# jondeaton/PhaMers

Hardware: AMD Instinct MI355X
Metric: Gbases/s k-mer-count+score, k=4, 5 kb contigs (higher is better)
Workload: dtype u32 counts + f16 MFMA proposal (exact integer counts x fp16 reference parts, f32 accumulate; k=4: high parts in the sweep, low parts added in f64 to the window's candidates) + f64 decision; 1 GPU; BASELINE configs[1]: k=4, 1000000 x 5000-base contigs per GPU, count+normalise+combo score, 4510 reference rows + 172 centroids; contigs_per_gpu=1000000, contig_length=5000, k=4, method=combo, parallelism=contig shards, 1 rank(s), replicated reference, final all-gather of scores

## Files before the change

### phamers_amd/csrc/count_slots.hip

```cpp
#include "count_shared.h"


__global__ __launch_bounds__(256) void phk_count_plan_kernel(const uint64_t *__restrict__ offsets, uint64_t n, int k,
                                                             uint32_t gs,
                                                             uint32_t long_thr, uint32_t piece_w, int sort,
                                                             uint32_t *__restrict__ ctl, uint32_t *__restrict__ ctl_next,
                                                             uint32_t *__restrict__ z0, uint32_t z0n, uint32_t *__restrict__ z1, uint32_t z1n) {
    __shared__ uint32_t h[SORT_KEYS];
    __shared__ unsigned long long s_pad[4], s_used[4];
    __shared__ uint32_t s_last;
    const int tid = threadIdx.x;
    {
        const uint32_t g0 = blockIdx.x * 256u + (uint32_t)tid, gn = gridDim.x * 256u;
        for (uint32_t i = g0; i < (uint32_t)CTL_WORDS; i += gn) ctl_next[i] = 0;
        for (uint32_t i = g0; i < z0n; i += gn) z0[i] = 0;
        for (uint32_t i = g0; i < z1n; i += gn) z1[i] = 0;
    }
    if (sort)
        for (int i = tid; i < SORT_KEYS; i += 256) h[i] = 0;
    __syncthreads();
    unsigned long long pad = 0, used = 0;
    for (uint64_t base = (uint64_t)blockIdx.x * PLAN_PER_BLOCK; base < n; base += (uint64_t)gridDim.x * PLAN_PER_BLOCK) {
        uint64_t o0[PLAN_PER_BLOCK / 256], o1[PLAN_PER_BLOCK / 256];
#pragma unroll
        for (int it = 0; it < PLAN_PER_BLOCK / 256; ++it) {
            const uint64_t c = base + (uint64_t)it * 256 + tid;
            const uint64_t cc = c < n ? c : n - 1;
            o0[it] = offsets[cc];
            o1[it] = offsets[cc + 1];
        }
#pragma unroll
        for (int it = 0; it < PLAN_PER_BLOCK / 256; ++it) {
            const uint64_t c = base + (uint64_t)it * 256 + tid;
            const bool have = c < n;
            uint64_t w = 0;
            if (have) {
                const uint64_t len = o1[it] - o0[it];
                w = len >= (uint64_t)k ? len - k + 1 : 0;
            }
            const unsigned long long wq = (have && w <= long_thr) ? w : 0ull;
            used += wq;
            unsigned long long mx = wq;
            for (uint32_t sft = 1; sft < gs; sft <<= 1) {
                const unsigned long long o = __shfl_xor(mx, (int)sft);
                mx = o > mx ? o : mx;
            }
            if (have && (c % gs) == 0) pad += (unsigned long long)gs * (((mx + 1023) >> 10) << 10);
            if (sort) {
                const uint32_t np = (have && w > long_thr && piece_w) ? (uint32_t)((w + piece_w - 1) / piece_w) : 1u;
                const uint32_t key = phk_windows_key(phk_piece_windows(w, np, np - 1, piece_w));
                const unsigned long long live = __ballot(have);
                const uint32_t key0 = __builtin_amdgcn_readfirstlane(key);
                if (__all(!have || (key == key0 && np == 1)) && (live & 1ull)) {
                    if ((tid & 63) == 0) atomicAdd(&h[key0], (uint32_t)__popcll(live));
                } else if (have) {
                    if (np > 1) atomicAdd(&h[phk_windows_key(piece_w)], np - 1);
                    atomicAdd(&h[key], 1u);
                }
            }
        }
    }
#pragma unroll
    for (int sft = 32; sft > 0; sft >>= 1) {
        pad += __shfl_xor(pad, sft);
        used += __shfl_xor(used, sft);
    }
    if ((tid & 63) == 0) {
        s_pad[tid >> 6] = pad;
        s_used[tid >> 6] = used;
    }
    __syncthreads();
    unsigned long long *stats = reinterpret_cast<unsigned long long *>(ctl + CTL_STATS);
    if (tid == 0) {
        pad = s_pad[0] + s_pad[1] + s_pad[2] + s_pad[3];
        used = s_used[0] + s_used[1] + s_used[2] + s_used[3];
        if (pad) {
            atomicAdd(stats, pad);
            atomicAdd(stats + 1, used);
        }
    }
    if (sort)
        for (int i = tid; i < SORT_KEYS; i += 256)
            if (h[i]) atomicAdd(ctl + CTL_CURSOR + i, h[i]);
    asm volatile("s_waitcnt vmcnt(0)" ::: "memory");
    __syncthreads();
    if (tid == 0) s_last = atomicAdd(ctl + CTL_TICKET, 1u) == gridDim.x - 1 ? 1u : 0u;
    __syncthreads();
    if (!s_last || !sort) return;
    const unsigned long long pad_t = __hip_atomic_load(stats, __ATOMIC_RELAXED, __HIP_MEMORY_SCOPE_AGENT);
    const unsigned long long used_t = __hip_atomic_load(stats + 1, __ATOMIC_RELAXED, __HIP_MEMORY_SCOPE_AGENT);
    if (used_t * 10ull >= pad_t * 6ull) return;
    for (int i = tid; i < SORT_KEYS; i += 256)
        h[i] = __hip_atomic_load(ctl + CTL_CURSOR + (SORT_KEYS - 1 - i), __ATOMIC_RELAXED, __HIP_MEMORY_SCOPE_AGENT);
    __syncthreads();
    if (tid < 64) {
        uint32_t loc = 0;
        for (int i = 0; i < SORT_KEYS / 64; ++i) loc += h[tid * (SORT_KEYS / 64) + i];
        uint32_t inc = loc;
#pragma unroll
        for (int sft = 1; sft < 64; sft <<= 1) {
            const uint32_t o = __shfl_up(inc, sft);
            if (tid >= sft) inc += o;
        }
        uint32_t run = inc - loc;
        for (int i = 0; i < SORT_KEYS / 64; ++i) {
            const uint32_t cnt = h[tid * (SORT_KEYS / 64) + i];
            h[tid * (SORT_KEYS / 64) + i] = run;
            run += cnt;
        }
        if (tid == 63) ctl[CTL_ITEMS] = run;
    }
    __syncthreads();
    for (int i = tid; i < SORT_KEYS; i += 256) ctl[CTL_CURSOR + (SORT_KEYS - 1 - i)] = h[i];
}

__global__ __launch_bounds__(256) void phk_sort_scatter_kernel(const uint64_t *__restrict__ offsets, uint64_t n, int k,
                                                               uint32_t long_thr, uint32_t piece_w,
                                                               const unsigned long long *__restrict__ stats,
                                                               uint32_t *__restrict__ cursor, uint2 *__restrict__ items,
                                                               uint32_t *__restrict__ counts, uint32_t *__restrict__ nwin) {
    if (phk_slots_apply(stats)) return;
    __shared__ uint32_t h[SORT_KEYS];
    const uint64_t per_block = (n + gridDim.x - 1) / gridDim.x;
    const uint64_t lo = per_block * blockIdx.x, hi = lo + per_block < n ? lo + per_block : n;
    const uint64_t D = 1ull << (2 * k);
    for (int i = threadIdx.x; i < SORT_KEYS; i += blockDim.x) h[i] = 0;
    __syncthreads();
    for (uint64_t c = lo + threadIdx.x; c < hi; c += blockDim.x) {
        uint32_t np;
        const uint64_t w = phk_contig_windows(offsets, c, k, long_thr, piece_w, np);
        if (np > 1) atomicAdd(&h[phk_windows_key(piece_w)], np - 1);
        atomicAdd(&h[phk_windows_key(phk_piece_windows(w, np, np - 1, piece_w))], 1u);
    }
    __syncthreads();
    for (int i = threadIdx.x; i < SORT_KEYS; i += blockDim.x)
        if (h[i]) h[i] = atomicAdd(cursor + i, h[i]);
    __syncthreads();
    for (uint64_t c = lo + threadIdx.x; c < hi; c += blockDim.x) {
        uint32_t np;
        const uint64_t w = phk_contig_windows(offsets, c, k, long_thr, piece_w, np);
        for (uint32_t pc = 0; pc < np; ++pc)
            items[atomicAdd(&h[phk_windows_key(phk_piece_windows(w, np, pc, piece_w))], 1u)] = make_uint2((uint32_t)c, pc);
        if (np > 1) {
            uint4 *row = reinterpret_cast<uint4 *>(counts + c * D);
            for (uint64_t i = 0; i < D / 4; ++i) row[i] = make_uint4(0, 0, 0, 0);
            if (nwin) nwin[c] = 0;
        }
    }
}


template <int NTH>
__global__ __launch_bounds__(NTH) void phk_count_pairs_kernel(const uint32_t *__restrict__ packed, const uint64_t *__restrict__ offsets,
                                                             uint64_t n, uint64_t max_word, uint32_t long_thr,
                                                             uint32_t *__restrict__ counts, uint32_t *__restrict__ nwin,
                                                             uint2 *__restrict__ long_list, uint32_t *__restrict__ long_count,
                                                             uint32_t piece_w) {
    constexpr int K = 4;
    constexpr uint32_t D = 256, NWORD = 512;
    constexpr int SLOTS = 32;
    constexpr int PARTS = NTH / SLOTS;
    constexpr int XPT = (int)D / PARTS;
    static_assert(XPT % 4 == 0, "flush geometry");
    extern __shared__ __attribute__((aligned(16))) uint32_t lds[];
    uint32_t *single_s = lds + NWORD * SLOTS;
    if (!phk_slots_apply(reinterpret_cast<const unsigned long long *>(long_count + CTL_STATS))) return;
    const int t = threadIdx.x;
    const int slot = t & (SLOTS - 1), part = t / SLOTS;
    for (uint32_t b = t * 4; b < NWORD * SLOTS; b += 4 * NTH) *reinterpret_cast<uint4 *>(lds + b) = make_uint4(0, 0, 0, 0);
    __syncthreads();
    const uint32_t colb = (uint32_t)slot * 4u;
    const uint32_t pthr = long_thr < 131070u ? long_thr : 131070u;
    typedef __attribute__((address_space(3))) uint32_t lds_u32;
    auto pair_addr = [&](uint32_t src, int o) { return (lds_u32 *)(uintptr_t)(((src >> (16 - 2 * o)) & (0x1FFu << 7)) | colb); };
    auto pair_inc = [&](uint32_t src, int o) {
        uint32_t bit, inc;
        asm("v_bfe_u32 %0, %1, %2, 1" : "=v"(bit) : "v"(src), "n"(22 - 2 * o));
        asm("v_mad_u32_u24 %0, %1, %2, 1" : "=v"(inc) : "v"(bit), "v"(65535u));
        return inc;
    };
#if defined(PHK_DIAGNOSTIC_BUILD) && defined(PAIRS_ABL) && PAIRS_ABL == 1
    auto add1 = [&](lds_u32 *p, uint32_t val) { asm volatile("" ::"v"(p), "v"(val)); };
#else
    auto add1 = [&](lds_u32 *p, uint32_t val) { __hip_atomic_fetch_add(p, val, __ATOMIC_RELAXED, __HIP_MEMORY_SCOPE_WORKGROUP); };
#endif
    const uint64_t wlast = max_word + 1;

    for (uint64_t batch = blockIdx.x; batch * SLOTS < n; batch += gridDim.x) {
        const uint64_t c = batch * SLOTS + slot;
        const bool have = c < n;
        const uint64_t st = have ? offsets[c] : 0;
        const uint64_t en = have ? offsets[c + 1] : 0;
        const uint64_t len = en - st;
        uint32_t W = len >= (uint64_t)K ? (uint32_t)((len - K + 1) < 0xFFFFFFFFull ? (len - K + 1) : 0xFFFFFFFFull) : 0;
        const bool handed_over = W > pthr;
        if (handed_over) {
            if (part == 0) {
                const uint32_t np = piece_w ? (W + piece_w - 1) / piece_w : 1u;
                const uint32_t base = atomicAdd(long_count, np);
                for (uint32_t pc = 0; pc < np; ++pc) long_list[base + pc] = make_uint2((uint32_t)c, pc);
            }
            W = 0;
        }
        const uint32_t par = (uint32_t)st & 1u;
        const uint32_t npair = W >> 1;
        const uint64_t U0 = st >> 6;
        const uint32_t rst = (uint32_t)(st - (U0 << 6));
        const uint32_t rPL = rst + 2u * npair - 2u;
        const uint32_t nunit = npair ? (rPL >> 6) + 1u : 0u;
        const uint32_t *pc = packed + 4 * U0;
        const uint32_t wlim = (uint32_t)((wlast - 4 * U0) < 0x7FFFFFFFull ? (wlast - 4 * U0) : 0x7FFFFFFFull);
        if (part == 0) {
            uint32_t sg = 0xFFFFFFFFu;
            if (W & 1u) {
                const uint64_t lb = st + W - 1, wl = lb >> 4;
                const uint64_t f = ((uint64_t)packed[wl] << 32) | packed[wl + 1];
                sg = (uint32_t)(f >> (56 - 2 * (uint32_t)(lb & 15))) & 0xFFu;
            }
            single_s[slot] = sg;
        }
        auto load5 = [&](uint32_t j, uint32_t (&w)[5]) {
            const uint32_t w0 = 4u * j;
            if (w0 + 3 <= wlim) {
                const uint4 a = *reinterpret_cast<const uint4 *>(pc + w0);
                w[0] = a.x; w[1] = a.y; w[2] = a.z; w[3] = a.w;
            } else {
                w[0] = pc[w0]; w[1] = pc[w0 + 1 < wlim ? w0 + 1 : wlim]; w[2] = pc[w0 + 2 < wlim ? w0 + 2 : wlim]; w[3] = pc[wlim];
            }
            w[4] = pc[w0 + 4 < wlim ? w0 + 4 : wlim];
        };
        uint32_t cur[5] = {0, 0, 0, 0, 0}, nxt[5] = {0, 0, 0, 0, 0};
        uint32_t j = (uint32_t)part;
        if (j < nunit) load5(j, cur);
        while (__any(j < nunit)) {
            const bool live = j < nunit;
            if (j + PARTS < nunit) load5(j + PARTS, nxt);
            const uint32_t s0 = 64u * j + par;
            const bool all = live && s0 >= rst && s0 + 62u <= rPL;
            uint32_t sw[5];
#pragma unroll
            for (int i = 0; i < 4; ++i) sw[i] = par ? __builtin_amdgcn_alignbit(cur[i], cur[i + 1], 30) : cur[i];
            sw[4] = par ? cur[4] << 2 : cur[4];
            if (!__any(live && !all)) {
                if (all) {
#pragma unroll
                    for (int wd = 0; wd < 4; ++wd) {
                        const uint32_t y = sw[wd], u = __builtin_amdgcn_alignbit(y, sw[wd + 1], 16);
#pragma unroll
                        for (int jp = 0; jp < 8; ++jp) {
                            const uint32_t src = jp < 5 ? y : u;
                            const int o = jp < 5 ? 2 * jp : 2 * jp - 8;
                            add1(pair_addr(src, o), pair_inc(src, o));
                        }
                    }
                }
            } else if (live) {
                const uint32_t ilo = rst > s0 ? (rst - s0) >> 1 : 0u;
                const uint32_t ihi = (rPL - s0) >> 1 < 31u ? (rPL - s0) >> 1 : 31u;
                const uint32_t pm = (ihi - ilo == 31u) ? ~0u : (((1u << (ihi - ilo + 1)) - 1u) << (31 - ihi));
#pragma unroll
                for (int wd = 0; wd < 4; ++wd) {
                    const uint32_t y = sw[wd], u = __builtin_amdgcn_alignbit(y, sw[wd + 1], 16);
#pragma unroll
                    for (int jp = 0; jp < 8; ++jp) {
                        const uint32_t src = jp < 5 ? y : u;
                        const int o = jp < 5 ? 2 * jp : 2 * jp - 8;
                        add1(pair_addr(src, o), pair_inc(src, o) * __builtin_amdgcn_ubfe(pm, 31 - (8 * wd + jp), 1));
                    }
                }
            }
#pragma unroll
            for (int i = 0; i < 5; ++i) cur[i] = nxt[i];
            j += PARTS;
        }
        phk_lds_barrier();
        {
            const uint32_t x0 = (uint32_t)part * XPT;
            uint32_t out[XPT];
            const uint32_t *col = lds + slot;
#pragma unroll
            for (int i = 0; i < XPT; ++i) {
                const uint32_t w0 = col[(2 * (x0 + i)) * SLOTS], w1 = col[(2 * (x0 + i) + 1) * SLOTS];
                out[i] = __builtin_amdgcn_sad_u16(w1, 0u, __builtin_amdgcn_sad_u16(w0, 0u, 0u));
            }
            const uint32_t one = 1u;
#pragma unroll
            for (int mm = 0; mm < XPT / 2; ++mm)
#pragma unroll
                for (int a = 0; a < 4; ++a) {
                    const uint32_t w = col[(128 * a + x0 / 2 + mm) * SLOTS];
                    asm("v_mad_u32_u16 %0, %1, %2, %0" : "+v"(out[2 * mm]) : "v"(w), "v"(one));
                    asm("v_mad_u32_u16 %0, %1, %2, %0 op_sel:[1,0,0,0]" : "+v"(out[2 * mm + 1]) : "v"(w), "v"(one));
                }
            const uint32_t sg = single_s[slot];
#pragma unroll
            for (int i = 0; i < XPT; ++i) out[i] += (sg == x0 + i) ? 1u : 0u;
            phk_lds_barrier();
            uint32_t *zc = lds + (2 * x0) * SLOTS + slot;
#pragma unroll
            for (int i = 0; i < 2 * XPT; ++i) zc[i * SLOTS] = 0;
            uint32_t *rowo = counts + c * D + x0;
#if defined(PHK_DIAGNOSTIC_BUILD) && defined(PAIRS_ABL) && PAIRS_ABL == 2
            if (have && (!handed_over || piece_w) && (batch & 63) == 0) {
#else
            if (have && (!handed_over || piece_w)) {
#endif
#pragma unroll
                for (int i = 0; i < XPT / 4; ++i)
                    *reinterpret_cast<uint4 *>(rowo + 4 * i) = make_uint4(out[4 * i], out[4 * i + 1], out[4 * i + 2], out[4 * i + 3]);
            }
            if (nwin && have && part == 0 && (!handed_over || piece_w)) nwin[c] = W;
        }
        phk_lds_barrier();
    }
}

template <int K, int SLOTS, int NTH, bool MASK, bool ORDERED>
__global__ __launch_bounds__(NTH) void phk_count_direct_kernel(const uint32_t *__restrict__ packed, const uint32_t *__restrict__ mask,
                                                              const uint64_t *__restrict__ offsets,
                                                              uint64_t n, uint64_t max_word, uint32_t long_thr,
                                                              uint32_t *__restrict__ counts, uint32_t *__restrict__ nwin,
                                                              uint2 *__restrict__ long_list, uint32_t *__restrict__ long_count,
                                                              const uint2 *__restrict__ order,
                                                              uint32_t piece_w,
                                                              uint32_t skip_plain,
                                                              uint4 *__restrict__ frag8,
                                                              uint32_t *__restrict__ big8) {
    constexpr uint32_t D = 1u << (2 * K);
    constexpr int PARTS = NTH / SLOTS;
    constexpr int XPT = (int)D / PARTS;
    constexpr int SHB = SLOTS == 32 ? 7 : 6;
    static_assert(XPT % 4 == 0 && K <= 5, "flush geometry / window fits the funnel");
    extern __shared__ __attribute__((aligned(16))) uint32_t lds[];
    uint32_t *nwin_s = lds + D * SLOTS;
    uint32_t *split_s = nwin_s + SLOTS;
    const bool plain = phk_slots_apply(reinterpret_cast<const unsigned long long *>(long_count + CTL_STATS));
    if (ORDERED) {
        if (plain || !order) return;
        n = long_count[CTL_ITEMS];
        frag8 = nullptr;
        big8 = nullptr;
    } else {
        if (!plain) {
            if (big8 && blockIdx.x == 0 && threadIdx.x == 0) big8[n] = 2u;
            return;
        }
        if (skip_plain) return;
        order = nullptr;
    }
    const int t = threadIdx.x;
    const int slot = t & (SLOTS - 1), part = t / SLOTS;
    for (uint32_t b = t * 4; b < D * SLOTS; b += 4 * NTH) *reinterpret_cast<uint4 *>(lds + b) = make_uint4(0, 0, 0, 0);
    if (t < SLOTS) nwin_s[t] = 0;
    __syncthreads();
    const uint32_t colb = (uint32_t)slot * 4u;
    typedef __attribute__((address_space(3))) uint32_t lds_u32;
    auto bin = [&](uint32_t src, int o) {
        constexpr uint32_t msk = (D - 1u) << SHB;
        const int sh = 32 - 2 * K - 2 * o - SHB;
        return (lds_u32 *)(uintptr_t)(((src >> sh) & msk) | colb);
    };
    auto add1 = [&](lds_u32 *p, uint32_t val) { __hip_atomic_fetch_add(p, val, __ATOMIC_RELAXED, __HIP_MEMORY_SCOPE_WORKGROUP); };
    const uint64_t wlast = max_word + 1;
    const uint64_t mlast = (max_word >> 1) + 1;

    for (uint64_t batch = blockIdx.x; batch * SLOTS < n; batch += gridDim.x) {
        const uint64_t ci = batch * SLOTS + slot;
        const bool have = ci < n;
        const uint2 item = (ORDERED && have) ? order[ci] : make_uint2(0, 0);
        const uint64_t c = have ? (ORDERED ? (uint64_t)item.x : ci) : 0;
        uint64_t st = have ? offsets[c] : 0;
        const uint64_t en = have ? offsets[c + 1] : 0;
        const uint64_t len = en - st;
        uint32_t W = len >= (uint64_t)K ? (uint32_t)((len - K + 1) < 0xFFFFFFFFull ? (len - K + 1) : 0xFFFFFFFFull) : 0;
        const bool split = ORDERED && piece_w && W > long_thr;
        if (split) {
            const uint64_t first = (uint64_t)item.y * piece_w;
            st += first;
            W = (uint32_t)((uint64_t)W - first < piece_w ? (uint64_t)W - first : piece_w);
        }
        const bool handed_over = !ORDERED && W > long_thr;
        if (ORDERED && part == 0) split_s[slot] = split ? (uint32_t)c + 1u : 0u;
        if (handed_over) {
            if (part == 0) {
                const uint32_t np = piece_w ? (W + piece_w - 1) / piece_w : 1u;
                const uint32_t base = atomicAdd(long_count, np);
                for (uint32_t pc = 0; pc < np; ++pc) long_list[base + pc] = make_uint2((uint32_t)c, pc);
            }
            W = 0;
        }
        const uint64_t U0 = st >> 6;
        const uint32_t rst = (uint32_t)(st - (U0 << 6));
        const uint64_t rlast64 = (uint64_t)rst + W - 1;
        const uint32_t rlast = rlast64 < 0xFFFFFFC0ull ? (uint32_t)rlast64 : 0xFFFFFFC0u;
        const uint32_t nunit = W ? (rlast >> 6) + 1u : 0u;
        const uint32_t *pc = packed + 4 * U0;
        const uint32_t wlim = (uint32_t)((wlast - 4 * U0) < 0x7FFFFFFFull ? (wlast - 4 * U0) : 0x7FFFFFFFull);
        const uint32_t *pm = MASK ? mask + 2 * U0 : nullptr;
        const uint32_t mlim = MASK ? (uint32_t)((mlast - 2 * U0) < 0x7FFFFFFFull ? (mlast - 2 * U0) : 0x7FFFFFFFull) : 0u;
        auto load5 = [&](uint32_t j, uint32_t (&w)[5], uint32_t (&mk)[3]) {
            const uint32_t w0 = 4u * j;
            if (w0 + 3 <= wlim) {
                const uint4 a = *reinterpret_cast<const uint4 *>(pc + w0);
                w[0] = a.x; w[1] = a.y; w[2] = a.z; w[3] = a.w;
            } else {
                w[0] = pc[w0]; w[1] = pc[w0 + 1 < wlim ? w0 + 1 : wlim]; w[2] = pc[w0 + 2 < wlim ? w0 + 2 : wlim]; w[3] = pc[wlim];
            }
            w[4] = pc[w0 + 4 < wlim ? w0 + 4 : wlim];
            if (MASK) {
#pragma unroll
                for (int i = 0; i < 3; ++i) mk[i] = pm[2 * j + i < mlim ? 2 * j + i : mlim];
            }
        };
        uint32_t cur[5] = {0, 0, 0, 0, 0}, nxt[5] = {0, 0, 0, 0, 0}, mcur[3] = {0, 0, 0}, mnxt[3] = {0, 0, 0};
        uint32_t cnt_ok = 0;
        uint32_t j = (uint32_t)part;
        if (j < nunit) load5(j, cur, mcur);
        while (__any(j < nunit)) {
            const bool live = j < nunit;
            if (j + PARTS < nunit) load5(j + PARTS, nxt, mnxt);
            const uint32_t fb = 64u * j;
            bool all = live && fb >= rst && fb + 63u <= rlast;
            uint64_t wv = 0;
            if (MASK ? live : (live && !all)) {
                const uint32_t lo = rst > fb ? rst - fb : 0u;
                const uint32_t hi = rlast - fb < 63u ? rlast - fb : 63u;
                wv = (hi - lo == 63u) ? ~0ull : (((1ull << (hi - lo + 1)) - 1ull) << (63 - hi));
                if (MASK) {
                    const uint64_t vb = ((uint64_t)mcur[0] << 32) | mcur[1];
                    uint64_t w = vb;
#pragma unroll
                    for (int jj = 1; jj < K; ++jj) w &= (vb << jj) | ((uint64_t)mcur[2] >> (32 - jj));
                    wv &= w;
                    all = all && w == ~0ull;
                    cnt_ok += (uint32_t)__popcll(wv);
                }
            }
            if (!__any(live && !all)) {
                if (all) {
#pragma unroll
                    for (int wd = 0; wd < 4; ++wd) {
                        const uint32_t y = cur[wd], u = __builtin_amdgcn_alignbit(y, cur[wd + 1], 16);
#pragma unroll
                        for (int jw = 0; jw < 16; ++jw) add1(bin(jw < 8 ? y : u, jw & 7), 1u);
                    }
                }
            } else if (live) {
                if (!MASK && all) wv = ~0ull;
                const uint32_t vhi = (uint32_t)(wv >> 32), vlo = (uint32_t)wv;
#pragma unroll
                for (int wd = 0; wd < 4; ++wd) {
                    const uint32_t y = cur[wd], u = __builtin_amdgcn_alignbit(y, cur[wd + 1], 16);
#pragma unroll
                    for (int jw = 0; jw < 16; ++jw) {
                        const int wi = 16 * wd + jw;
                        add1(bin(jw < 8 ? y : u, jw & 7), __builtin_amdgcn_ubfe(wi < 32 ? vhi : vlo, 31 - (wi & 31), 1));
                    }
                }
            }
#pragma unroll
            for (int i = 0; i < 5; ++i) cur[i] = nxt[i];
            if (MASK) {
#pragma unroll
                for (int i = 0; i < 3; ++i) mcur[i] = mnxt[i];
            }
            j += PARTS;
        }
        if (MASK && cnt_ok) atomicAdd(nwin_s + slot, cnt_ok);
        phk_lds_barrier();
        if (ORDERED) {
            for (int sl = t >> 6; sl < SLOTS; sl += NTH / 64) {
                const uint32_t cs = split_s[sl];
                if (!cs) continue;
                uint32_t *rowp = counts + (uint64_t)(cs - 1u) * D;
                for (uint32_t code = (uint32_t)(t & 63); code < D; code += 64) {
                    const uint32_t v = lds[code * SLOTS + sl];
                    if (v) atomicAdd(rowp + code, v);
                }
            }
            phk_lds_barrier();
        }
        {
            uint32_t *cellb = lds + ((uint32_t)part * XPT) * SLOTS + slot;
            uint32_t *rowo = counts + c * D + (uint32_t)part * XPT;
            const uint32_t Wc = MASK ? nwin_s[slot] : W;
            const int cen = (int)phk_row_center(Wc, D);
            uint32_t mx = 0, l1 = 0;
            constexpr int PZ = XPT >= 16 ? XPT / 16 : 1, CPZ = XPT >= 16 ? 4 : XPT / 4;
#pragma unroll
            for (uint32_t pz = 0; pz < (uint32_t)PZ; ++pz) {
                uint32_t pk[4] = {0, 0, 0, 0};
#pragma unroll
                for (uint32_t i = 0; i < (uint32_t)CPZ; ++i) {
                    uint32_t *cell = cellb + (16 * pz + 4 * i) * SLOTS;
                    const uint4 o = make_uint4(cell[0], cell[SLOTS], cell[2 * SLOTS], cell[3 * SLOTS]);
                    cell[0] = 0; cell[SLOTS] = 0; cell[2 * SLOTS] = 0; cell[3 * SLOTS] = 0;
                    if (!split && have && (!handed_over || piece_w)) *reinterpret_cast<uint4 *>(rowo + 16 * pz + 4 * i) = o;
                    if (XPT >= 16) {
                        const uint32_t cc[4] = {o.x, o.y, o.z, o.w};
                        uint32_t word = 0;
#pragma unroll
                        for (int b = 0; b < 4; ++b) {
                            const int d = (int)cc[b] - cen;
                            const uint32_t ad = (uint32_t)(d < 0 ? -d : d);
                            mx = max(mx, ad);
                            l1 += min(ad, 127u);
                            const int q = d < -127 ? -127 : (d > 127 ? 127 : d);
                            word |= ((uint32_t)q & 0xFFu) << (8 * b);
                        }
                        pk[i] = word;
                    }
                }
                if (XPT >= 16 && frag8 && have && !handed_over) {
                    const uint32_t dim16 = (uint32_t)part * PZ + pz;
                    frag8[((c >> 5) * (D / 32) + (dim16 >> 1)) * 64 + 32u * (dim16 & 1u) + (uint32_t)(c & 31)] = make_uint4(pk[0], pk[1], pk[2], pk[3]);
                }
            }
            if (big8 && have) {
                if (handed_over) {
                    if (part == 0) {
                        big8[c] = PHK_PREP8_MISSING;
                        atomicOr(big8 + n, 1u);
                    }
                } else {
                    if (mx > 127u) atomicOr(big8 + c, 0x80000000u);
                    if (2ull * Wc + D > PHK_I8_L1_MAX) atomicAdd(big8 + c, l1);
                }
            }
            if (nwin && have && part == 0) {
                if (split) atomicAdd(nwin + c, Wc);
                else if (!handed_over || piece_w) nwin[c] = Wc;
            }
        }
        phk_lds_barrier();
        if (MASK) {
            if (t < SLOTS) nwin_s[t] = 0;
            phk_lds_barrier();
        }
    }
}

typedef void (*PairsKern)(const uint32_t *, const uint64_t *, uint64_t, uint64_t, uint32_t, uint32_t *, uint32_t *, uint2 *, uint32_t *,
                          uint32_t);
typedef void (*DirectKern)(const uint32_t *, const uint32_t *, const uint64_t *, uint64_t, uint64_t, uint32_t, uint32_t *, uint32_t *,
                           uint2 *, uint32_t *, const uint2 *, uint32_t, uint32_t, uint4 *, uint32_t *);
struct PairsShape {
    unsigned threads;
    PairsKern kern;
};
struct DirectShape {
    int k;
    unsigned slots, threads;
    DirectKern kern[2][2];
};
#define DIRECT_SHAPE(K_, S_, T_)                                                                                  \
    {K_, S_, T_, {{phk_count_direct_kernel<K_, S_, T_, false, false>, phk_count_direct_kernel<K_, S_, T_, false, true>}, \
                  {phk_count_direct_kernel<K_, S_, T_, true, false>, phk_count_direct_kernel<K_, S_, T_, true, true>}}}
static const PairsShape PAIRS_SHAPES[] = {{512, phk_count_pairs_kernel<512>}, {1024, phk_count_pairs_kernel<1024>}};
static const DirectShape DIRECT_SHAPES[] = {DIRECT_SHAPE(3, 32, 512), DIRECT_SHAPE(4, 32, 512), DIRECT_SHAPE(4, 32, 1024),
                                            DIRECT_SHAPE(5, 16, 512), DIRECT_SHAPE(5, 16, 1024)};
#undef DIRECT_SHAPE

static int slots_instance_init(const void *kern, bool *ok) {
    PHK_HIP(hipFuncSetAttribute(kern, hipFuncAttributeMaxDynamicSharedMemorySize, 96 * 1024));
    hipFuncAttributes fa;
    PHK_HIP(hipFuncGetAttributes(&fa, kern));
    if (fa.sharedSizeBytes != 0) *ok = false;
    return PHK_OK;
}

int phk_count_init_device(phk_ctx *ctx) {
    bool ok = true;
    for (const PairsShape &p : PAIRS_SHAPES) PHK_TRY(slots_instance_init((const void *)p.kern, &ok));
    for (const DirectShape &d : DIRECT_SHAPES)
        for (int i = 0; i < 4; ++i) PHK_TRY(slots_instance_init((const void *)d.kern[i >> 1][i & 1], &ok));
    ctx->slots_lds0 = ok;
    return PHK_OK;
}

int phk_launch_count_plan(phk_ctx *ctx, const CountRoute &r, const CountCall &c, const PhkStepLink *link) {
    PHK_LAUNCH(ctx, "phk_count_plan_kernel",
               phk_count_plan_kernel<<<dim3(r.plan_blocks), dim3(256), 0, ctx->stream>>>(
                   c.offsets, r.plan_n, r.k, r.slots, r.long_thr, r.piece_w, r.sorted ? 1 : 0, c.ctl, c.ctl_next,
                   link ? link->zero[0] : nullptr, link ? link->zero_words[0] : 0u, link ? link->zero[1] : nullptr,
                   link ? link->zero_words[1] : 0u));
    return PHK_OK;
}

int phk_launch_sort_scatter(phk_ctx *ctx, const CountRoute &r, const CountCall &c) {
    PHK_LAUNCH(ctx, "phk_sort_scatter_kernel",
               phk_sort_scatter_kernel<<<dim3(r.sort_blocks), dim3(256), 0, ctx->stream>>>(
                   c.offsets, r.n, r.k, r.long_thr, r.piece_w, (const unsigned long long *)(c.ctl + CTL_STATS), c.ctl + CTL_CURSOR,
                   c.order, c.counts, c.nwin));
    return PHK_OK;
}

int phk_launch_count_pairs(phk_ctx *ctx, const CountRoute &r, const CountCall &c) {
    for (const PairsShape &p : PAIRS_SHAPES) {
        if (p.threads != r.pairs_threads) continue;
        PHK_LAUNCH(ctx, "phk_count_pairs_kernel",
                   p.kern<<<dim3(phk_count_grid(ctx, r.pairs_groups, r.pairs_per_cu)), dim3(p.threads), r.pairs_lds, ctx->stream>>>(
                       c.packed, c.offsets, r.n, r.max_word, r.long_thr, c.counts, c.nwin, c.long_list, c.ctl, r.piece_w));
        return PHK_OK;
    }
    phk_set_error("phk_count: no two-windows-per-add kernel of %u threads", r.pairs_threads);
    return PHK_ERR_UNSUPPORTED;
}

int phk_launch_count_direct(phk_ctx *ctx, const CountRoute &r, const CountCall &c, PhkStepLink *link) {
    const bool prep = r.k == 5 && !r.masked && link && link->prep8.offered && link->prep8.counts == c.counts && link->prep8.n == r.n &&
                      link->prep8.D == 1024;
    uint4 *frag8 = prep ? (uint4 *)link->prep8.frag : nullptr;
    uint32_t *big8 = prep ? link->prep8.big : nullptr;
    if (link) link->prep8.written = prep;
    for (const DirectShape &d : DIRECT_SHAPES) {
        if (d.k != r.k || d.threads != r.direct_threads) continue;
        const unsigned blocks = phk_count_grid(ctx, r.direct_groups, r.direct_per_cu);
        for (int ordered = 0; ordered < 2; ++ordered) {
            if (ordered ? !r.sorted : r.skip_plain) continue;
            PHK_LAUNCH(ctx, "phk_count_direct_kernel",
                       d.kern[r.masked][ordered]<<<dim3(blocks), dim3(d.threads), r.direct_lds, ctx->stream>>>(
                           c.packed, c.mask, c.offsets, r.n, r.max_word, r.long_thr, c.counts, c.nwin, c.long_list, c.ctl, c.order,
                           r.piece_w, r.skip_plain ? 1u : 0u, frag8, big8));
        }
        return PHK_OK;
    }
    phk_set_error("phk_count: no slot kernel for k = %d with %u threads", r.k, r.direct_threads);
    return PHK_ERR_UNSUPPORTED;
}
```

Before: 1480 Gbases/s.

## Prefetch next batch offsets and first words, repack pair-count increments

Moves the load of the next batch's contig offsets, first packed words and single-tail words so they are issued during the current batch's flush, overlapping global latency with LDS reduction work. The pair histogram increment encoding changes from 65535/1 to a 65536-scaled form, with a subtract-based decode in the flush. Increments are now computed from pre-masked 16-bit lanes with v_mad_u32_u16, which feeds two atomics per source word. The alignbit parity shift is skipped when no lane in the wave has odd parity. This adds register pressure for the prefetched state and makes the count encoding harder to verify.

```diff
diff --git a/phamers_amd/csrc/count_slots.hip b/phamers_amd/csrc/count_slots.hip
--- a/phamers_amd/csrc/count_slots.hip
+++ b/phamers_amd/csrc/count_slots.hip
@@ -176,7 +176,20 @@
     auto pair_inc = [&](uint32_t src, int o) {
         uint32_t bit, inc;
         asm("v_bfe_u32 %0, %1, %2, 1" : "=v"(bit) : "v"(src), "n"(22 - 2 * o));
-        asm("v_mad_u32_u24 %0, %1, %2, 1" : "=v"(inc) : "v"(bit), "v"(65535u));
+        asm("v_mad_u32_u24 %0, %1, %2, 1" : "=v"(inc) : "v"(bit), "v"(65536u));
+        return inc;
+    };
+    const uint32_t sel_scale = 1024u;
+    auto half_addr = [&](uint32_t idx, bool hi) {
+        uint32_t a;
+        if (hi) asm("v_mad_u32_u16 %0, %1, 1, %2 op_sel:[1,0,0,0]" : "=v"(a) : "v"(idx), "v"(colb));
+        else asm("v_mad_u32_u16 %0, %1, 1, %2" : "=v"(a) : "v"(idx), "v"(colb));
+        return (lds_u32 *)(uintptr_t)a;
+    };
+    auto half_inc = [&](uint32_t sel, bool hi) {
+        uint32_t inc;
+        if (hi) asm("v_mad_u32_u16 %0, %1, %2, 1 op_sel:[1,0,0,0]" : "=v"(inc) : "v"(sel), "s"(sel_scale));
+        else asm("v_mad_u32_u16 %0, %1, %2, 1" : "=v"(inc) : "v"(sel), "s"(sel_scale));
         return inc;
     };
 #if defined(PHK_DIAGNOSTIC_BUILD) && defined(PAIRS_ABL) && PAIRS_ABL == 1
@@ -185,72 +198,111 @@
     auto add1 = [&](lds_u32 *p, uint32_t val) { __hip_atomic_fetch_add(p, val, __ATOMIC_RELAXED, __HIP_MEMORY_SCOPE_WORKGROUP); };
 #endif
     const uint64_t wlast = max_word + 1;
+    struct Geo {
+        uint32_t W, Wc;
+        uint32_t rst, rPL;
+        uint32_t nunit, wlim;
+        const uint32_t *pc;
+    };
+    auto geometry = [&](uint64_t st, uint64_t en) {
+        Geo g;
+        const uint64_t len = en - st;
+        g.W = len >= (uint64_t)K ? (uint32_t)((len - K + 1) < 0xFFFFFFFFull ? (len - K + 1) : 0xFFFFFFFFull) : 0;
+        g.Wc = g.W > pthr ? 0u : g.W;
+        const uint32_t npair = g.Wc >> 1;
+        const uint64_t U0 = st >> 6;
+        g.rst = (uint32_t)(st - (U0 << 6));
+        g.rPL = g.rst + 2u * npair - 2u;
+        g.nunit = npair ? (g.rPL >> 6) + 1u : 0u;
+        g.pc = packed + 4 * U0;
+        g.wlim = (uint32_t)((wlast - 4 * U0) < 0x7FFFFFFFull ? (wlast - 4 * U0) : 0x7FFFFFFFull);
+        return g;
+    };
+    auto load5 = [&](const Geo &g, uint32_t j, uint32_t (&w)[5]) {
+        const uint32_t *pc = g.pc;
+        const uint32_t wlim = g.wlim, w0 = 4u * j;
+        if (w0 + 3 <= wlim) {
+            const uint4 a = *reinterpret_cast<const uint4 *>(pc + w0);
+            w[0] = a.x; w[1] = a.y; w[2] = a.z; w[3] = a.w;
+        } else {
+            w[0] = pc[w0]; w[1] = pc[w0 + 1 < wlim ? w0 + 1 : wlim]; w[2] = pc[w0 + 2 < wlim ? w0 + 2 : wlim]; w[3] = pc[wlim];
+        }
+        w[4] = pc[w0 + 4 < wlim ? w0 + 4 : wlim];
+    };
+    uint64_t st_n = 0, en_n = 0;
+    uint32_t cur[5] = {0, 0, 0, 0, 0}, sgw[2] = {0, 0};
+    auto request_offsets = [&](uint64_t b) {
+        const uint64_t cn = b * SLOTS + slot;
+        const bool hn = cn < n;
+        st_n = hn ? offsets[cn] : 0;
+        en_n = hn ? offsets[cn + 1] : 0;
+    };
+    auto request_first = [&](uint64_t st, const Geo &g) {
+        if ((uint32_t)part < g.nunit) load5(g, (uint32_t)part, cur);
+        if (part == 0 && (g.Wc & 1u)) {
+            const uint64_t wl = (st + g.Wc - 1) >> 4;
+            sgw[0] = packed[wl];
+            sgw[1] = packed[wl + 1];
+        }
+    };
+    if ((uint64_t)blockIdx.x * SLOTS < n) {
+        request_offsets(blockIdx.x);
+        request_first(st_n, geometry(st_n, en_n));
+    }
 
     for (uint64_t batch = blockIdx.x; batch * SLOTS < n; batch += gridDim.x) {
-        const uint64_t c = batch * SLOTS + slot;
+        uint64_t bcur = batch, bnext = batch + gridDim.x;
+        asm volatile("" : "+s"(bcur), "+s"(bnext));
+        const uint64_t c = bcur * SLOTS + slot;
         const bool have = c < n;
-        const uint64_t st = have ? offsets[c] : 0;
-        const uint64_t en = have ? offsets[c + 1] : 0;
-        const uint64_t len = en - st;
-        uint32_t W = len >= (uint64_t)K ? (uint32_t)((len - K + 1) < 0xFFFFFFFFull ? (len - K + 1) : 0xFFFFFFFFull) : 0;
-        const bool handed_over = W > pthr;
-        if (handed_over) {
-            if (part == 0) {
-                const uint32_t np = piece_w ? (W + piece_w - 1) / piece_w : 1u;
-                const uint32_t base = atomicAdd(long_count, np);
-                for (uint32_t pc = 0; pc < np; ++pc) long_list[base + pc] = make_uint2((uint32_t)c, pc);
-            }
-            W = 0;
+        const uint64_t st = st_n, en = en_n;
+        const bool more = (batch + gridDim.x) * SLOTS < n;
+        const Geo g = geometry(st, en);
+        const uint32_t W = g.Wc;
+        const bool handed_over = g.W > pthr;
+        if (handed_over && part == 0) {
+            const uint32_t np = piece_w ? (g.W + piece_w - 1) / piece_w : 1u;
+            const uint32_t base = atomicAdd(long_count, np);
+            for (uint32_t pc = 0; pc < np; ++pc) long_list[base + pc] = make_uint2((uint32_t)c, pc);
         }
         const uint32_t par = (uint32_t)st & 1u;
-        const uint32_t npair = W >> 1;
-        const uint64_t U0 = st >> 6;
-        const uint32_t rst = (uint32_t)(st - (U0 << 6));
-        const uint32_t rPL = rst + 2u * npair - 2u;
-        const uint32_t nunit = npair ? (rPL >> 6) + 1u : 0u;
-        const uint32_t *pc = packed + 4 * U0;
-        const uint32_t wlim = (uint32_t)((wlast - 4 * U0) < 0x7FFFFFFFull ? (wlast - 4 * U0) : 0x7FFFFFFFull);
+        const uint32_t rst = g.rst, rPL = g.rPL, nunit = g.nunit;
         if (part == 0) {
             uint32_t sg = 0xFFFFFFFFu;
             if (W & 1u) {
-                const uint64_t lb = st + W - 1, wl = lb >> 4;
-                const uint64_t f = ((uint64_t)packed[wl] << 32) | packed[wl + 1];
+                const uint64_t lb = st + W - 1;
+                const uint64_t f = ((uint64_t)sgw[0] << 32) | sgw[1];
                 sg = (uint32_t)(f >> (56 - 2 * (uint32_t)(lb & 15))) & 0xFFu;
             }
             single_s[slot] = sg;
         }
-        auto load5 = [&](uint32_t j, uint32_t (&w)[5]) {
-            const uint32_t w0 = 4u * j;
-            if (w0 + 3 <= wlim) {
-                const uint4 a = *reinterpret_cast<const uint4 *>(pc + w0);
-                w[0] = a.x; w[1] = a.y; w[2] = a.z; w[3] = a.w;
-            } else {
-                w[0] = pc[w0]; w[1] = pc[w0 + 1 < wlim ? w0 + 1 : wlim]; w[2] = pc[w0 + 2 < wlim ? w0 + 2 : wlim]; w[3] = pc[wlim];
-            }
-            w[4] = pc[w0 + 4 < wlim ? w0 + 4 : wlim];
-        };
-        uint32_t cur[5] = {0, 0, 0, 0, 0}, nxt[5] = {0, 0, 0, 0, 0};
+        uint32_t nxt[5] = {0, 0, 0, 0, 0};
         uint32_t j = (uint32_t)part;
-        if (j < nunit) load5(j, cur);
+        const bool any_odd = __any(par);
         while (__any(j < nunit)) {
             const bool live = j < nunit;
-            if (j + PARTS < nunit) load5(j + PARTS, nxt);
+            if (j + PARTS < nunit) load5(g, j + PARTS, nxt);
             const uint32_t s0 = 64u * j + par;
             const bool all = live && s0 >= rst && s0 + 62u <= rPL;
             uint32_t sw[5];
 #pragma unroll
-            for (int i = 0; i < 4; ++i) sw[i] = par ? __builtin_amdgcn_alignbit(cur[i], cur[i + 1], 30) : cur[i];
-            sw[4] = par ? cur[4] << 2 : cur[4];
+            for (int i = 0; i < 5; ++i) sw[i] = cur[i];
+            if (any_odd) {
+#pragma unroll
+                for (int i = 0; i < 4; ++i) sw[i] = par ? __builtin_amdgcn_alignbit(cur[i], cur[i + 1], 30) : cur[i];
+                sw[4] = par ? cur[4] << 2 : cur[4];
+            }
             if (!__any(live && !all)) {
                 if (all) {
 #pragma unroll
                     for (int wd = 0; wd < 4; ++wd) {
-                        const uint32_t y = sw[wd], u = __builtin_amdgcn_alignbit(y, sw[wd + 1], 16);
-#pragma unroll
-                        for (int jp = 0; jp < 8; ++jp) {
-                            const uint32_t src = jp < 5 ? y : u;
-                            const int o = jp < 5 ? 2 * jp : 2 * jp - 8;
-                            add1(pair_addr(src, o), pair_inc(src, o));
+                        const uint32_t y = sw[wd], v = __builtin_amdgcn_alignbit(y, sw[wd + 1], 24);
+                        const uint32_t srcs[4] = {y, y << 4, v, v << 4};
+#pragma unroll
+                        for (int q = 0; q < 4; ++q) {
+                            const uint32_t idx = srcs[q] & 0xFF80FF80u, sel = srcs[q] & 0x00400040u;
+                            add1(half_addr(idx, true), half_inc(sel, true));
+                            add1(half_addr(idx, false), half_inc(sel, false));
                         }
                     }
                 }
@@ -273,28 +325,36 @@
             for (int i = 0; i < 5; ++i) cur[i] = nxt[i];
             j += PARTS;
         }
+        if (more) request_offsets(bnext);
         phk_lds_barrier();
         {
-            const uint32_t x0 = (uint32_t)part * XPT;
+            uint32_t x0 = (uint32_t)part * XPT;
+            asm volatile("" : "+v"(x0));
             uint32_t out[XPT];
             const uint32_t *col = lds + slot;
-#pragma unroll
-            for (int i = 0; i < XPT; ++i) {
-                const uint32_t w0 = col[(2 * (x0 + i)) * SLOTS], w1 = col[(2 * (x0 + i) + 1) * SLOTS];
-                out[i] = __builtin_amdgcn_sad_u16(w1, 0u, __builtin_amdgcn_sad_u16(w0, 0u, 0u));
-            }
             const uint32_t one = 1u;
 #pragma unroll
-            for (int mm = 0; mm < XPT / 2; ++mm)
+            for (int i = 0; i < XPT; ++i) out[i] = 0;
+#pragma unroll
+            for (int mm = 0; mm < XPT / 2; ++mm) {
 #pragma unroll
                 for (int a = 0; a < 4; ++a) {
                     const uint32_t w = col[(128 * a + x0 / 2 + mm) * SLOTS];
                     asm("v_mad_u32_u16 %0, %1, %2, %0" : "+v"(out[2 * mm]) : "v"(w), "v"(one));
                     asm("v_mad_u32_u16 %0, %1, %2, %0 op_sel:[1,0,0,0]" : "+v"(out[2 * mm + 1]) : "v"(w), "v"(one));
                 }
+                out[2 * mm] -= out[2 * mm + 1];
+            }
+#pragma unroll
+            for (int i = 0; i < XPT; ++i) {
+                const uint32_t w0 = col[(2 * (x0 + i)) * SLOTS], w1 = col[(2 * (x0 + i) + 1) * SLOTS];
+                asm("v_mad_u32_u16 %0, %1, %2, %0" : "+v"(out[i]) : "v"(w0), "v"(one));
+                asm("v_mad_u32_u16 %0, %1, %2, %0" : "+v"(out[i]) : "v"(w1), "v"(one));
+            }
             const uint32_t sg = single_s[slot];
 #pragma unroll
             for (int i = 0; i < XPT; ++i) out[i] += (sg == x0 + i) ? 1u : 0u;
+            if (more) request_first(st_n, geometry(st_n, en_n));
             phk_lds_barrier();
             uint32_t *zc = lds + (2 * x0) * SLOTS + slot;
 #pragma unroll
```

New measurement: 1476 Gbases/s. No clear change (-0.3%).
